# maciejkula/sbr-rs

Hardware: AMD Instinct MI355X
Metric: train interactions/sec (higher is better)
Workload: dtype f32

## Files before the change

### sbr_rs_amd/csrc/sbr_kernels.hip

```cpp

#include "sbr_kernels.h"

#include <atomic>
#include <cstdlib>
#include <cstring>

#include "../../include/sbr_hip.h"
#include "sbr_device.h"
#include "sbr_numerics.h"

namespace sbr {

typedef float f32x4 __attribute__((ext_vector_type(4)));
typedef unsigned v4u32 __attribute__((ext_vector_type(4)));

#define EWMA_CHUNK_SEQS 256
#ifndef SBR_FWD_RT
#define SBR_FWD_RT 4
#endif
#ifndef SBR_FWD_WPE
#define SBR_FWD_WPE 3
#endif
#define SBR_MAX_T 1024
#ifndef SBR_FWD_RT4_MIN_TILES
// ... 1378 lines not shown
        const __amdgpu_buffer_rsrc_t rsC = row_rsrc(w.C, D * 4, rb + b0, nr_live);
#pragma unroll
        for (int k = 0; k < CITER; ++k)
            dst[k] = __builtin_bit_cast(float4, __builtin_amdgcn_raw_buffer_load_b128(rsC, tid * 16, k * NT * 16, SBR_AUX_BWD_LD));
    };
    auto request_gates = [&](int t) {
        const int tid = thread_id();
        int rb, nr;
        step_rows(t, &rb, &nr);
        const __amdgpu_buffer_rsrc_t rsG = row_rsrc(w.G, 4 * D * 4, rb + b0, nr);
        const int vg = (tid / Q) * (4 * D * 4) + (tid % Q) * 16;
#pragma unroll
        for (int k = 0; k < CITER; ++k) {
            const int so = k * (NT / Q) * (4 * D * 4);
#pragma unroll
            for (int g = 0; g < 4; ++g)
                pg[k][g] = __builtin_bit_cast(float4, __builtin_amdgcn_raw_buffer_load_b128(rsG, vg + g * D * 4, so, SBR_AUX_BWD_LD));
        }
    };

    f32x4 ring0[PF], ring1[PF];
    const __amdgpu_buffer_rsrc_t wrs = __builtin_amdgcn_make_buffer_rsrc((void*)m.WTp, (short)0, 2 * D * NGD * 4, SBR_BUFFER_RSRC_FLAGS);
    const uint32_t lane_byte = (uint32_t)(tid0 & 63) * 16u;
    auto load_ring = [&](int slot, int S) {
        ring0[slot] = __builtin_bit_cast(f32x4, __builtin_amdgcn_raw_buffer_load_b128(wrs, lane_byte, (wv * NSZ + S) * 1024, 0));
        ring1[slot] = __builtin_bit_cast(f32x4, __builtin_amdgcn_raw_buffer_load_b128(wrs, lane_byte, ((UT + wv) * NSZ + S) * 1024, 0));
    };
    const int ts = nsteps - 1;
    request_ids(ts);
    request_gates(ts);
    request_cstate(pc, ts);
    request_cstate(pcp, ts > 0 ? ts - 1 : 0);
    request_gathers(ts);
    if (ts > 0) request_ids(ts - 1);
#pragma unroll
    for (int j = 0; j < PF; ++j) load_ring(j, j);

#ifdef SBR_PROF_BWD
    long long bprof[8] = {0, 0, 0, 0, 0, 0, 0, 0};
#define BPROF(k_) { const long long now_ = clock64(); bprof[k_] += now_ - bprof_t; bprof_t = now_; }
    long long bprof_t = clock64();
#else
#define BPROF(k_)
#endif
    auto step = [&](int t) {
        int row_begin, nrows, nrows_above = 0;
        step_rows(t, &row_begin, &nrows);
        if (t + 1 < nsteps) { int rb_; step_rows(t + 1, &rb_, &nrows_above); }
        BPROF(0)
        __syncthreads();
        BPROF(1)
        {
            const int tid = thread_id();
            const __amdgpu_buffer_rsrc_t rsZ = row_rsrc(w.dZ, NGD * 4, row_begin + b0, nrows);
            const int vz = (tid / Q) * (NGD * 4) + (tid % Q) * 16;
#pragma unroll
            for (int k = 0; k < CITER; ++k) {
                const int idx = tid + k * NT;
                const int i = idx / Q;
                const int u = (idx % Q) * 4;
                const bool carried = i < nrows_above;
                const float2 r01 = *reinterpret_cast<const float2*>(&Zs[i * LDZ + u]);
                const float2 r23 = *reinterpret_cast<const float2*>(&Zs[i * LDZ + u + 2]);
                const float recv[4] = {carried ? r01.x : 0.0f, carried ? r01.y : 0.0f, carried ? r23.x : 0.0f, carried ? r23.y : 0.0f};
                const float g_ = pcoef[k];
                const float dhl[4] = {g_ * pen[k].x - g_ * pep[k].x, g_ * pen[k].y - g_ * pep[k].y,
                                      g_ * pen[k].z - g_ * pep[k].z, g_ * pen[k].w - g_ * pep[k].w};
                const float gi[4] = {pg[k][0].x, pg[k][0].y, pg[k][0].z, pg[k][0].w};
                const float gf[4] = {pg[k][1].x, pg[k][1].y, pg[k][1].z, pg[k][1].w};
                const float gg[4] = {pg[k][2].x, pg[k][2].y, pg[k][2].z, pg[k][2].w};
                const float go[4] = {pg[k][3].x, pg[k][3].y, pg[k][3].z, pg[k][3].w};
                const float cc[4] = {pc[k].x, pc[k].y, pc[k].z, pc[k].w};
                const float cp[4] = {pcp[k].x, pcp[k].y, pcp[k].z, pcp[k].w};
                float dz[4][4];
#pragma unroll
                for (int j = 0; j < 4; ++j) {
                    const float dh = dhl[j] + recv[j];
                    float dco;
                    sbr_lstm_cell_bwd(dh, carried ? dc[k][j] : 0.0f, gi[j], gf[j], gg[j], go[j], cc[j], t > 0 ? cp[j] : 0.0f, NG == 3,
                                      &dz[0][j], &dz[1][j], &dz[2][j], &dz[3][j], &dco);
                    dc[k][j] = dco;
                }
#pragma unroll
                for (int g = 0; g < NG; ++g) {
                    const int src = NG == 4 ? g : g + 1;
                    __builtin_amdgcn_raw_buffer_store_b128(__builtin_bit_cast(v4u32, make_float4(dz[src][0], dz[src][1], dz[src][2], dz[src][3])), rsZ,
                                                           vz + g * D * 4, k * (NT / Q) * (NGD * 4), SBR_AUX_BWD_Z);
                    float2* dst = reinterpret_cast<float2*>(&Zs[i * LDZ + g * D + u]);
                    dst[0] = make_float2(dz[src][0], dz[src][1]);
                    dst[1] = make_float2(dz[src][2], dz[src][3]);
                }
            }
        }
        BPROF(2)
        __syncthreads();
        BPROF(3)
        const int tid = thread_id();
        const int lane = tid & 63;
        const int c16 = lane & 15;
        const int kq = lane >> 4;
        f32x4 acc[2][RT];
#pragma unroll
        for (int cc = 0; cc < 2; ++cc)
#pragma unroll
            for (int rt = 0; rt < RT; ++rt) acc[cc][rt] = (f32x4){0.f, 0.f, 0.f, 0.f};
        float av[RT][4];
        auto read_a = [&](int S) {
#pragma unroll
            for (int rt = 0; rt < RT; ++rt) {
                const float* arow = &Zs[(rt * 16 + c16) * LDZ + 16 * (S < NSZ ? S : NSZ - 1) + kq];
                av[rt][0] = arow[0]; av[rt][1] = arow[4]; av[rt][2] = arow[8]; av[rt][3] = arow[12];
            }
        };
        read_a(0);
        auto mma_block = [&](int S, int slot) {
            float ac[RT][4];
#pragma unroll
            for (int rt = 0; rt < RT; ++rt)
#pragma unroll
                for (int sub = 0; sub < 4; ++sub) ac[rt][sub] = av[rt][sub];
            read_a(S + 1);
#pragma unroll
            for (int sub = 0; sub < 4; ++sub)
#pragma unroll
                for (int rt = 0; rt < RT; ++rt) {
                    acc[0][rt] = __builtin_amdgcn_mfma_f32_16x16x4f32(ac[rt][sub], ring0[slot][sub], acc[0][rt], 0, 0, 0);
                    acc[1][rt] = __builtin_amdgcn_mfma_f32_16x16x4f32(ac[rt][sub], ring1[slot][sub], acc[1][rt], 0, 0, 0);
                }
        };
#pragma unroll
        for (int j = 0; j < PF; ++j) {
            mma_block(j, j);
            __builtin_amdgcn_sched_barrier(0);
            load_ring(j, j + PF);
            __builtin_amdgcn_sched_barrier(0);
        }
        if (t > 0) {
            request_gathers(t - 1);
            request_ids(t > 1 ? t - 2 : 0);
        }
        __builtin_amdgcn_sched_barrier(0);
#pragma unroll 1
        for (int S0 = PF; S0 < NSZ - PF; S0 += PF) {
#pragma unroll
            for (int j = 0; j < PF; ++j) {
                mma_block(S0 + j, j);
                __builtin_amdgcn_sched_barrier(0);
                load_ring(j, S0 + j + PF);
                __builtin_amdgcn_sched_barrier(0);
            }
        }
#pragma unroll
        for (int j = 0; j < PF; ++j) {
            mma_block(NSZ - PF + j, j);
            __builtin_amdgcn_sched_barrier(0);
        }
        {
            const int tn = t > 0 ? t - 1 : 0;
#pragma unroll
            for (int k = 0; k < CITER; ++k) pc[k] = pcp[k];
            request_gates(tn);
            request_cstate(pcp, tn > 0 ? tn - 1 : 0);
        }
        BPROF(4)
        __syncthreads();
        BPROF(5)
        {
            const __amdgpu_buffer_rsrc_t rsX = row_rsrc(blk.dX, D * 4, row_begin + b0, nrows);
            const int vx = (kq * 4 * D + wv * 16 + c16) * 4;
#pragma unroll
            for (int rt = 0; rt < RT; ++rt)
#pragma unroll
                for (int reg = 0; reg < 4; ++reg) {
                    const int i = rt * 16 + kq * 4 + reg;
                    const float dx = acc[0][rt][reg];
                    __builtin_amdgcn_raw_buffer_store_b32(__builtin_bit_cast(unsigned, dx), rsX, vx, (rt * 16 + reg) * D * 4, SBR_AUX_BWD_ST);
                    Zs[i * LDZ + wv * 16 + c16] = acc[1][rt][reg];
                }
        }
#pragma unroll
        for (int j = 0; j < PF; ++j) load_ring(j, j);
    };
    step(ts);
#pragma unroll 1
    for (int t = ts - 1; t >= 0; --t) step(t);
#ifdef SBR_PROF_BWD
    if ((tile == 20 || tile == 350) && (tid0 & 63) == 0 && (wv == 0 || wv == 5))
        printf("BWDPROF tile %d wave %d steps %d per-step cycles: epilogue+ringreq %lld barA %lld cell %lld barB %lld gemm+requests %lld barC %lld\n", tile, wv,
               nsteps, bprof[0] / nsteps, bprof[1] / nsteps, bprof[2] / nsteps, bprof[3] / nsteps, bprof[4] / nsteps, bprof[5] / nsteps);
#endif
}

template <int D, int NG>
__global__ __launch_bounds__(256) void lstm_dw_kernel(ModelView m, MbView mb, BlockView blk, WorkView w) {
    constexpr int K2 = 2 * D;
    constexpr int NGD = NG * D;
    constexpr int TJ = (NGD + 127) / 128;
    constexpr int SLAB = 32;
    __shared__ float Xs[SLAB * 128];
    __shared__ float Zs[SLAB * 128];
    __shared__ int s_prev[SBR_DW_CHUNK_ROWS];
    const int tid = threadIdx.x;
    const int lane = tid & 63;
    const int wave = __builtin_amdgcn_readfirstlane(tid >> 6);
    const int wk = wave >> 1, wj = wave & 1;
    constexpr int NTILE = ((K2 + 127) / 128) * TJ;
    const int wid = blockIdx.x;
    const int tile = (wid >> 3) % NTILE;
    const int c = (wid >> 3) / NTILE * 8 + (wid & 7);
    if (c * SBR_DW_CHUNK_ROWS >= mb.R) return;
    const int tk = tile / TJ, tj = tile % TJ;
    const int r0 = c * SBR_DW_CHUNK_ROWS;
    int r1 = r0 + SBR_DW_CHUNK_ROWS;
    if (r1 > mb.R) r1 = mb.R;
    const int nr = r1 - r0;
    for (int i = tid; i < nr; i += 256) {
        s_prev[i] = mb.prev_row[r0 + i];
    }
    __syncthreads();
    const int l31 = lane & 31;
    const int hh = lane >> 5;
    f32x16 acc[2][2];
#pragma unroll
    for (int a = 0; a < 2; ++a)
#pragma unroll
        for (int b = 0; b < 2; ++b)
#pragma unroll
            for (int q = 0; q < 16; ++q) acc[a][b][q] = 0.0f;
    const int c4 = (tid & 31) * 4;
    const int srow = tid >> 5;
    const int kcol = tk * 128 + c4;
    const int jcol = tj * 128 + c4;
    float4 xr[4], zr[4];
    auto fetch = [&](int slab) {
#pragma unroll
        for (int i = 0; i < 4; ++i) {
            const int lr = slab * SLAB + srow + 8 * i;
            float4 xv = make_float4(0.f, 0.f, 0.f, 0.f), zv = make_float4(0.f, 0.f, 0.f, 0.f);
            if (lr < nr) {
                if (kcol < D) xv = ld4(w.X + (size_t)(r0 + lr) * D + kcol);
                else if (kcol < K2) {
                    const int pr = s_prev[lr];
                    if (pr >= 0) xv = ld4(blk.H + (size_t)pr * D + (kcol - D));
                }
                if (jcol < NGD) zv = ld4(w.dZ + (size_t)(r0 + lr) * NGD + jcol);
            }
            xr[i] = xv;
            zr[i] = zv;
        }
    };
    const int nslabs = (nr + SLAB - 1) / SLAB;
    float bias_acc = 0.0f;
    const bool do_bias = tk == 0 && tid < 128 && tj * 128 + tid < NGD;
    fetch(0);
    for (int slab = 0; slab < nslabs; ++slab) {
#pragma unroll
        for (int i = 0; i < 4; ++i) {
            st4(&Xs[(srow + 8 * i) * 128 + c4], xr[i]);
            st4(&Zs[(srow + 8 * i) * 128 + c4], zr[i]);
        }
        __syncthreads();
        if (slab + 1 < nslabs) fetch(slab + 1);
        const float* xa = &Xs[hh * 128 + wk * 64 + l31];
        const float* zb = &Zs[hh * 128 + wj * 64 + l31];
#pragma unroll 4
        for (int s = 0; s < SLAB / 2; ++s) {
            const float a0 = xa[s * 256], a1 = xa[s * 256 + 32];
            const float b0 = zb[s * 256], b1 = zb[s * 256 + 32];
            acc[0][0] = __builtin_amdgcn_mfma_f32_32x32x2f32(a0, b0, acc[0][0], 0, 0, 0);
            acc[0][1] = __builtin_amdgcn_mfma_f32_32x32x2f32(a0, b1, acc[0][1], 0, 0, 0);
            acc[1][0] = __builtin_amdgcn_mfma_f32_32x32x2f32(a1, b0, acc[1][0], 0, 0, 0);
            acc[1][1] = __builtin_amdgcn_mfma_f32_32x32x2f32(a1, b1, acc[1][1], 0, 0, 0);
        }
        if (do_bias) {
            const int rows_here = nr - slab * SLAB < SLAB ? nr - slab * SLAB : SLAB;
            for (int r = 0; r < rows_here; ++r) bias_acc = bias_acc + Zs[r * 128 + tid];
        }
        __syncthreads();
    }
    if (do_bias) w.partials[((size_t)c * (K2 + 1) + K2) * NGD + tj * 128 + tid] = bias_acc;
    float* part = w.partials + (size_t)c * (K2 + 1) * NGD;
#pragma unroll
    for (int a = 0; a < 2; ++a)
#pragma unroll
        for (int b = 0; b < 2; ++b) {
            const int j = tj * 128 + wj * 64 + b * 32 + l31;
#pragma unroll
            for (int q = 0; q < 16; ++q) {
                const int k = tk * 128 + wk * 64 + a * 32 + (q & 3) + 8 * (q >> 2) + 4 * hh;
                if (k < K2 && j < NGD) part[(size_t)k * NGD + j] = acc[a][b][q];
            }
        }
}

template <int D, int NG>
__global__ __launch_bounds__(256, SBR_DW_WPE) void lstm_dw_full_kernel(ModelView m, MbView mb, BlockView blk, WorkView w) {
    constexpr int K2 = 2 * D;
    constexpr int NGD = NG * D;
    constexpr int TJ = NGD / 128;
    constexpr int SLAB = SBR_DW_SLAB;
    constexpr int NI = SLAB / 8;
    constexpr int NTILE = (K2 / 128) * TJ;
    static_assert(K2 % 128 == 0 && NGD % 128 == 0, "full tiles only");
    __shared__ float Xs[SLAB * 128];
    __shared__ float Zs[SLAB * 128];
    __shared__ int s_prev[SBR_DW_CHUNK_ROWS];
    const int tid = threadIdx.x;
    const int lane = tid & 63;
    const int wave = __builtin_amdgcn_readfirstlane(tid >> 6);
    const int wk = wave >> 1, wj = wave & 1;
    const int wid = blockIdx.x;
    const int tile = (wid >> 3) % NTILE;
    const int c = (wid >> 3) / NTILE * 8 + (wid & 7);
    if (c * SBR_DW_CHUNK_ROWS >= mb.R) return;
    const int tk = tile / TJ, tj = tile % TJ;
    const int r0 = c * SBR_DW_CHUNK_ROWS;
    const int last = mb.R - 1;
    for (int i = tid; i < SBR_DW_CHUNK_ROWS; i += 256) s_prev[i] = mb.prev_row[r0 + i <= last ? r0 + i : last];
    __syncthreads();
    const int l31 = lane & 31;
    const int hh = lane >> 5;
    f32x16 acc[2][2];
#pragma unroll
    for (int a = 0; a < 2; ++a)
#pragma unroll
        for (int b = 0; b < 2; ++b)
#pragma unroll
            for (int q = 0; q < 16; ++q) acc[a][b][q] = 0.0f;
    const int c4 = (tid & 31) * 4;
    const int srow = tid >> 5;
    const int kcol = tk * 128 + c4;
    const int jcol = tj * 128 + c4;
    const bool xpart = kcol < D;
    float4 xr[NI], zr[NI];
    const bool small_h = !w.wide_addresses && (size_t)mb.R * D * 4 < ((size_t)1 << 31);
    const int xrows = mb.R - r0 < SBR_DW_CHUNK_ROWS ? mb.R - r0 : SBR_DW_CHUNK_ROWS;
    const __amdgpu_buffer_rsrc_t rsZ = __builtin_amdgcn_make_buffer_rsrc((void*)(w.dZ + (size_t)r0 * NGD), (short)0, xrows * NGD * 4, SBR_BUFFER_RSRC_FLAGS);
    const __amdgpu_buffer_rsrc_t rsXc = __builtin_amdgcn_make_buffer_rsrc((void*)(w.X + (size_t)r0 * D), (short)0, xrows * D * 4, SBR_BUFFER_RSRC_FLAGS);
    const __amdgpu_buffer_rsrc_t rsH = __builtin_amdgcn_make_buffer_rsrc((void*)blk.H, (short)0, small_h ? (int)((size_t)mb.R * D * 4) : 0, SBR_BUFFER_RSRC_FLAGS);
    auto fetch = [&](int slab) {
        if (D >= 128 && small_h) {
#pragma unroll
            for (int i = 0; i < NI; ++i) {
                const int lr = slab * SLAB + srow + 8 * i;
                if (tk * 128 < D) {
                    xr[i] = __builtin_bit_cast(float4, __builtin_amdgcn_raw_buffer_load_b128(rsXc, (srow * D + kcol) * 4, (slab * SLAB + 8 * i) * D * 4, SBR_AUX_DW_LD));
                } else {
                    const int pr = s_prev[lr];
                    xr[i] = __builtin_bit_cast(float4, __builtin_amdgcn_raw_buffer_load_b128(rsH, pr >= 0 ? (int)((uint32_t)pr * (uint32_t)(D * 4) + (uint32_t)((kcol - D) * 4)) : -16, 0, 0));
                }
                zr[i] = __builtin_bit_cast(float4, __builtin_amdgcn_raw_buffer_load_b128(rsZ, (srow * NGD + jcol) * 4, (slab * SLAB + 8 * i) * NGD * 4, SBR_AUX_DW_LD));
            }
            return;
        }
        const float* X = launder(w.X);
        const float* H = launder(blk.H);
        const float* dZ = launder(w.dZ);
        const float* zero = launder(w.zeros);
#pragma unroll
        for (int i = 0; i < NI; ++i) {
            const int lr = slab * SLAB + srow + 8 * i;
            const int row = r0 + lr <= last ? r0 + lr : last;
            const int pr = s_prev[lr];
            const float* src = xpart ? X + ((size_t)row * D + kcol) : (pr >= 0 ? H + ((size_t)pr * D + (kcol - D)) : zero + (kcol - D));
            xr[i] = ld4(src);
            zr[i] = ld4(dZ + ((size_t)(r0 + lr) * NGD + jcol));
        }
    };
    int nr = mb.R - r0;
    nr = nr < SBR_DW_CHUNK_ROWS ? nr : SBR_DW_CHUNK_ROWS;
    const int nslabs = (nr + SLAB - 1) / SLAB;
    float bias_acc = 0.0f;
    const bool do_bias = tk == 0 && tid < 128;
    fetch(0);
    for (int slab = 0; slab < nslabs; ++slab) {
#pragma unroll
        for (int i = 0; i < NI; ++i) {
            st4(&Xs[(srow + 8 * i) * 128 + c4], xr[i]);
            st4(&Zs[(srow + 8 * i) * 128 + c4], zr[i]);
        }
        __syncthreads();
        fetch(slab + 1 < nslabs ? slab + 1 : slab);
        const float* xa = &Xs[hh * 128 + wk * 64 + l31];
        const float* zb = &Zs[hh * 128 + wj * 64 + l31];
        float a0 = xa[0], a1 = xa[32], b0 = zb[0], b1 = zb[32];
#pragma unroll
        for (int s = 0; s < SLAB / 2; ++s) {
            const int sn = s + 1 < SLAB / 2 ? s + 1 : s;
            const float na0 = xa[sn * 256], na1 = xa[sn * 256 + 32];
            const float nb0 = zb[sn * 256], nb1 = zb[sn * 256 + 32];
            acc[0][0] = __builtin_amdgcn_mfma_f32_32x32x2f32(a0, b0, acc[0][0], 0, 0, 0);
            acc[0][1] = __builtin_amdgcn_mfma_f32_32x32x2f32(a0, b1, acc[0][1], 0, 0, 0);
            acc[1][0] = __builtin_amdgcn_mfma_f32_32x32x2f32(a1, b0, acc[1][0], 0, 0, 0);
            acc[1][1] = __builtin_amdgcn_mfma_f32_32x32x2f32(a1, b1, acc[1][1], 0, 0, 0);
            a0 = na0; a1 = na1; b0 = nb0; b1 = nb1;
        }
        if (do_bias) {
            const int rows_here = nr - slab * SLAB < SLAB ? nr - slab * SLAB : SLAB;
            for (int r = 0; r < rows_here; ++r) bias_acc = bias_acc + Zs[r * 128 + tid];
        }
        __syncthreads();
    }
    if (do_bias) w.partials[((size_t)c * (K2 + 1) + K2) * NGD + tj * 128 + tid] = bias_acc;
    float* part = w.partials + (size_t)c * (K2 + 1) * NGD;
#pragma unroll
    for (int a = 0; a < 2; ++a)
#pragma unroll
        for (int b = 0; b < 2; ++b) {
            const int j = tj * 128 + wj * 64 + b * 32 + l31;
#pragma unroll
            for (int q = 0; q < 16; ++q) {
                const int k = tk * 128 + wk * 64 + a * 32 + (q & 3) + 8 * (q >> 2) + 4 * hh;
                part[(size_t)k * NGD + j] = acc[a][b][q];
            }
        }
}

__global__ void dense_reduce_local_kernel(const float* partials, int nchunks, size_t n, float* dense) {
    const size_t i = (size_t)blockIdx.x * blockDim.x + threadIdx.x;
    if (i >= n) return;
    float acc = partials[i];
    int c = 1;
    for (; c + 8 <= nchunks; c += 8) {
        float v[8];
#pragma unroll
        for (int j = 0; j < 8; ++j) v[j] = partials[(size_t)(c + j) * n + i];
#pragma unroll
        for (int j = 0; j < 8; ++j) acc = acc + v[j];
    }
    for (; c < nchunks; ++c) acc = acc + partials[(size_t)c * n + i];
    dense[i] = acc;
}

__device__ __forceinline__ size_t wp_index(int k, int jcol, int D, int NG) {
    const int K2 = 2 * D;
    const int g = jcol / D, u = jcol % D;
    const int ut = u >> 4, j16 = u & 15;
    const int S = k >> 4, sub = (k & 15) >> 2, kq = k & 3;
    const int lane = kq * 16 + j16;
    return ((((size_t)(ut * NG + g) * (K2 / 16) + S) * 64 + lane) * 4 + sub);
}
__device__ __forceinline__ size_t wtp_index(int k, int jcol, int D, int NG) {
    const int NGD = NG * D;
    const int ct = k >> 4, c16 = k & 15;
    const int S = jcol >> 4, sub = (jcol & 15) >> 2, kq = jcol & 3;
    const int lane = kq * 16 + c16;
    return ((((size_t)ct * (NGD / 16) + S) * 64 + lane) * 4 + sub);
}

__device__ __forceinline__ void dense_apply_element(const ModelView& m, size_t i, float g);
__global__ void dense_apply_kernel(ModelView m, const uint8_t* all_blocks, uint64_t block_bytes, uint64_t dense_off,
                                   int ndev, size_t n, const float* partials, int nchunks, float* dense_out) {
    const size_t i = (size_t)blockIdx.x * blockDim.x + threadIdx.x;
    if (i >= n) return;
    float g;
    if (partials) {
        g = partials[i];
        int c = 1;
        for (; c + 8 <= nchunks; c += 8) {
            float v[8];
#pragma unroll
            for (int j = 0; j < 8; ++j) v[j] = partials[(size_t)(c + j) * n + i];
#pragma unroll
            for (int j = 0; j < 8; ++j) g = g + v[j];
        }
        for (; c < nchunks; ++c) g = g + partials[(size_t)c * n + i];
        dense_out[i] = g;
    } else {
        g = reinterpret_cast<const float*>(all_blocks + dense_off)[i];
        for (int q = 1; q < ndev; ++q) g = g + reinterpret_cast<const float*>(all_blocks + (size_t)q * block_bytes + dense_off)[i];
    }
    dense_apply_element(m, i, g);
}
__device__ __forceinline__ void dense_apply_element(const ModelView& m, size_t i, float g) {
    if (m.ng) {
        const int NGD = m.ng * m.d;
        const size_t nw = (size_t)2 * m.d * NGD;
        if (i < nw) {
            const bool adam = m.optimizer == SBR_OPT_ADAM;
            float wv = m.W[i], G = m.Wacc[i], M = adam ? m.Wm[i] : 0.0f;
            opt_update(m, &wv, &G, &M, g);
            m.W[i] = wv;
            m.Wacc[i] = G;
            if (adam) m.Wm[i] = M;
            const int k = (int)(i / NGD), jcol = (int)(i % NGD);
            m.Wp[wp_index(k, jcol, m.d, m.ng)] = wv;
            m.WTp[wtp_index(k, jcol, m.d, m.ng)] = wv;
        } else {
            const size_t j = i - nw;
            const bool adam = m.optimizer == SBR_OPT_ADAM;
            float wv = m.bW[j], G = m.bWacc[j], M = adam ? m.bWm[j] : 0.0f;
            opt_update(m, &wv, &G, &M, g);
            m.bW[j] = wv;
            m.bWacc[j] = G;
            if (adam) m.bWm[j] = M;
        }
    } else {
        const bool adam = m.optimizer == SBR_OPT_ADAM;
        float wv = m.alpha[i], G = m.alpha_acc[i], M = adam ? m.alpha_m[i] : 0.0f;
        opt_update(m, &wv, &G, &M, g);
        m.alpha[i] = wv;
        m.alpha_acc[i] = G;
        if (adam) m.alpha_m[i] = M;
    }
}

__global__ void repack_lstm_kernel(ModelView m) {
    const int NGD = m.ng * m.d;
    const size_t nw = (size_t)2 * m.d * NGD;
    const size_t i = (size_t)blockIdx.x * blockDim.x + threadIdx.x;
    if (i >= nw) return;
    const int k = (int)(i / NGD), jcol = (int)(i % NGD);
    const float wv = m.W[i];
    m.Wp[wp_index(k, jcol, m.d, m.ng)] = wv;
    m.WTp[wtp_index(k, jcol, m.d, m.ng)] = wv;
}


struct UpdAccess {
    static __device__ __forceinline__ float4 ld(const float* p) { return ld4_upd(p); }
    static __device__ __forceinline__ void st(float* p, float4 v) { st4_upd(p, v); }
};
struct NoPrefetch {};
struct EmitApply {
    ModelView m;
    template <int D>
    __device__ __forceinline__ RowUpdate<D> pre(uint32_t r, int lg) const {
        RowUpdate<D> q;
        q.template load<UpdAccess>(m, r, lg);
        return q;
    }
    template <int D>
    __device__ __forceinline__ void row(uint32_t r, uint64_t, int lg, const RowSum& s, RowUpdate<D> q) const {
        q.apply(m, s);
        q.template store<UpdAccess>(m, r, lg);
        q.update_bias(m, r, lg, s);
    }
};
struct EmitChunk {
    void* send;
    uint64_t S;
    template <int D>
    __device__ __forceinline__ NoPrefetch pre(uint32_t, int) const { return NoPrefetch{}; }
    template <int D>
    __device__ __forceinline__ void row(uint32_t r, uint64_t, int lg, const RowSum& s, NoPrefetch) const {
        const uint32_t S32 = (uint32_t)S, owner = r / S32;
        float* c = reinterpret_cast<float*>(send) + (uint64_t)owner * S * ((uint64_t)D + 2);
        const uint64_t lr = r - owner * S32;
        st4(c + lr * D + 4 * lg, s.g);
        if (lg == 0) {
            if (s.has_b()) c[S * D + lr] = s.gb;
            reinterpret_cast<uint32_t*>(c + S * D + S)[lr] = 1u | (s.has_b() ? 2u : 0u);
        }
    }
};
struct EmitList {
    float* G;
    float* gbl;
    uint32_t* fl;
    template <int D>
    __device__ __forceinline__ NoPrefetch pre(uint32_t, int) const { return NoPrefetch{}; }
    template <int D>
    __device__ __forceinline__ void row(uint32_t, uint64_t p, int lg, const RowSum& s, NoPrefetch) const {
        st4(G + p * D + 4 * lg, s.g);
        if (lg == 0) {
            gbl[p] = s.gb;
            fl[p] = 1u | (s.has_b() ? 2u : 0u);
        }
    }
};

template <int D>
__device__ __forceinline__ RowSum seg_accumulate(const BlockView& blk, const uint64_t* keys, uint64_t begin, uint64_t end, int lg) {
    RowSum s;
    for (uint64_t e = begin; e < end; e += 4) {
        float4 v[4];
        float sc[4];
        bool bias[4];
#pragma unroll
        for (int i = 0; i < 4; ++i) {
            v[i] = make_float4(0.f, 0.f, 0.f, 0.f);
            sc[i] = 0.0f;
            bias[i] = false;
            if (e + i < end) {
                const EntrySource src = entry_source((uint32_t)keys[e + i]);
                v[i] = ld4(src.rows(blk.dX, blk.H) + (size_t)src.r * D + 4 * lg);
                sc[i] = src.scale_at(blk.coef);
                bias[i] = src.carries_bias();
            }
        }
#pragma unroll
        for (int i = 0; i < 4; ++i)
            if (e + i < end) s.add_entry(v[i], sc[i], bias[i]);
    }
    return s;
}

template <int D, int NB>
__device__ __forceinline__ RowSum seg_accumulate_long(const BlockView& blk, const uint64_t* keys, uint64_t begin, uint64_t end, int lg) {
    RowSum s;
    const uint32_t* klo = reinterpret_cast<const uint32_t*>(keys);
    uint32_t src_n[NB];
#pragma unroll
    for (int i = 0; i < NB; ++i) src_n[i] = begin + i < end ? klo[2 * (begin + i)] : 0u;
#pragma unroll 1
    for (uint64_t e = begin; e < end; e += NB) {
        float4 v[NB];
        float sc[NB];
        EntrySource src[NB];
#pragma unroll
        for (int i = 0; i < NB; ++i) {
            src[i] = entry_source(src_n[i]);
            v[i] = make_float4(0.f, 0.f, 0.f, 0.f);
            sc[i] = 0.0f;
            if (e + i < end) {
                v[i] = ld4(src[i].rows(blk.dX, blk.H) + (size_t)src[i].r * D + 4 * lg);
                sc[i] = blk.coef[src[i].r];
            }
        }
#pragma unroll
        for (int i = 0; i < NB; ++i) src_n[i] = e + NB + i < end ? klo[2 * (e + NB + i)] : 0u;
#pragma unroll
        for (int i = 0; i < NB; ++i)
            if (e + i < end) s.add_entry(v[i], src[i].scale(sc[i]), src[i].carries_bias());
    }
    return s;
}

__device__ __forceinline__ uint64_t seg_end(const uint64_t* keys, uint64_t lo, uint64_t hi, uint32_t row) {
    while (lo < hi) {
        const uint64_t mid = lo + (hi - lo) / 2;
        if ((uint32_t)(keys[mid] >> 32) == row) lo = mid + 1; else hi = mid;
    }
    return lo;
}

template <int D, class Emit, bool INLINE_LONG>
__device__ __forceinline__ void seg_short_rows(const BlockView& blk, const uint64_t* keys, uint64_t n, const SegScratch& sc, const Emit& emit,
                                               uint32_t wave, uint32_t nwaves) {
    const LaneGroup<D> lanes(wave, nwaves);
    constexpr int L = LaneGroup<D>::L;
    const int lg = lanes.lg, gbase = lanes.grp * L;
    const uint32_t nheads = *sc.nheads;
    const uint32_t stride = (uint32_t)lanes.stride;
    uint32_t h = (uint32_t)lanes.first();
    auto head_at = [&](uint32_t hh) { return sc.head_pos[hh < nheads ? hh : nheads]; };
    auto window_key = [&](uint32_t p0, uint32_t p1) {
        const uint32_t c = p1 - p0 < (uint32_t)L ? p1 - p0 : (uint32_t)L;
        return keys[(uint32_t)lg < c ? (uint64_t)p0 + lg : ((uint64_t)p0 < n ? (uint64_t)p0 : 0)];
    };
    uint32_t p_cur = head_at(h), p_end = head_at(h + 1);
    uint32_t p_next = head_at(h + stride), p_next_end = head_at(h + stride + 1);
    uint64_t kmine = window_key(p_cur, p_end);
    for (uint32_t h0 = (uint32_t)lanes.wave_first; h0 < nheads; h0 += stride, h += stride) {
        const bool active = h < nheads;
        const uint32_t p_nn = head_at(h + 2 * stride), p_nn_end = head_at(h + 2 * stride + 1);
        const uint64_t p = p_cur;
        const uint32_t len = active ? p_end - p_cur : 0u;
        const uint32_t cnt = len < (uint32_t)L ? len : (uint32_t)L;
        const uint32_t lo = (uint32_t)kmine;
        const uint32_t row = (uint32_t)__shfl((int)(uint32_t)(kmine >> 32), gbase, 64);
        kmine = window_key(p_next, p_next_end);
        p_cur = p_next;
        p_end = p_next_end;
        p_next = p_nn;
        p_next_end = p_nn_end;
        if (INLINE_LONG && len > SBR_SEG_CHUNK) {
            const auto pre = emit.template pre<D>(row, lg);
            RowSum s = seg_accumulate_long<D, 8>(blk, keys, p, p + SBR_SEG_CHUNK, lg);
            for (uint64_t q = p + SBR_SEG_CHUNK; q < p + len; q += SBR_SEG_CHUNK)
                s.add_partial(seg_accumulate_long<D, 8>(blk, keys, q, q + SBR_SEG_CHUNK < p + len ? q + SBR_SEG_CHUNK : p + len, lg));
            emit.template row<D>(row, p, lg, s, pre);
            continue;
        }
        if (!INLINE_LONG && len > SBR_SEG_ROUTE) {
            if (lg == 0 && !sc.prelisted) {
                const uint32_t slot = atomicAdd(&sc.counters[0], 1u);
                if (slot < sc.cap) {
                    sc.long_start[slot] = (uint32_t)p;
                    sc.long_end[slot] = (uint32_t)p + len;
                }
            }
            continue;
        }
        if (!active) continue;
        const auto pre = emit.template pre<D>(row, lg);
        RowSum s;
        if (len <= (uint32_t)L) {
            for (int e = 0; e < (int)cnt; e += 4) {
                float4 v[4];
                float scl[4];
                bool bias[4];
#pragma unroll
                for (int i = 0; i < 4; ++i) {
                    v[i] = make_float4(0.f, 0.f, 0.f, 0.f);
                    scl[i] = 0.0f;
                    bias[i] = false;
                    if (e + i < (int)cnt) {
                        const EntrySource src = entry_source((uint32_t)__shfl((int)lo, gbase + e + i, 64));
                        v[i] = ld4(src.rows(blk.dX, blk.H) + (size_t)src.r * D + 4 * lg);
                        scl[i] = src.scale_at(blk.coef);
                        bias[i] = src.carries_bias();
                    }
                }
#pragma unroll
                for (int i = 0; i < 4; ++i)
                    if (e + i < (int)cnt) s.add_entry(v[i], scl[i], bias[i]);
            }
        } else {
            s = seg_accumulate<D>(blk, keys, p, p + len, lg);
        }
        emit.template row<D>(row, p, lg, s, pre);
    }
}
template <int D, class Emit, bool INLINE_LONG = false>
__global__ __launch_bounds__(256) void seg_short_kernel(BlockView blk, const uint64_t* keys, uint64_t n, SegScratch sc, Emit emit) {
    seg_short_rows<D, Emit, INLINE_LONG>(blk, keys, n, sc, emit, (uint32_t)((blockIdx.x * (uint64_t)blockDim.x + threadIdx.x) >> 6),
                                         (uint32_t)(((uint64_t)gridDim.x * blockDim.x) >> 6));
// ... 881 lines not shown
```

Before: 108.6 million.

## Switch LSTM dW kernel to 16x16x4 MFMA with padded LDS rows

Replaces the 2x2 grid of 32x32x2 f32 MFMAs in the full-tile LSTM weight-gradient kernel with a 4x4 grid of 16x16x4 MFMAs that consume four k-rows per step. LDS rows are padded to a stride of 144 floats so fragment reads avoid bank conflicts, and the output store is rewritten to match the new accumulator layout. It also adds optional compile-time scheduling barriers and a hoisted bias reduction. The goal is higher MFMA throughput and fewer LDS conflicts, at the cost of more accumulator registers and more shared memory.

After: 109.1 million (median of 6 runs). About the same (+0.4%).

```diff
diff --git a/sbr_rs_amd/csrc/sbr_kernels.hip b/sbr_rs_amd/csrc/sbr_kernels.hip
--- a/sbr_rs_amd/csrc/sbr_kernels.hip
+++ b/sbr_rs_amd/csrc/sbr_kernels.hip
@@ -1704,8 +1704,10 @@
     constexpr int NI = SLAB / 8;
     constexpr int NTILE = (K2 / 128) * TJ;
     static_assert(K2 % 128 == 0 && NGD % 128 == 0, "full tiles only");
-    __shared__ float Xs[SLAB * 128];
-    __shared__ float Zs[SLAB * 128];
+    constexpr int LD = 144;
+    static_assert(SLAB % 4 == 0 && LD % 32 == 16, "whole k-blocks per slab; conflict-free fragment reads");
+    __shared__ float Xs[SLAB * LD];
+    __shared__ float Zs[SLAB * LD];
     __shared__ int s_prev[SBR_DW_CHUNK_ROWS];
     const int tid = threadIdx.x;
     const int lane = tid & 63;
@@ -1720,15 +1722,15 @@
     const int last = mb.R - 1;
     for (int i = tid; i < SBR_DW_CHUNK_ROWS; i += 256) s_prev[i] = mb.prev_row[r0 + i <= last ? r0 + i : last];
     __syncthreads();
-    const int l31 = lane & 31;
-    const int hh = lane >> 5;
-    f32x16 acc[2][2];
-#pragma unroll
-    for (int a = 0; a < 2; ++a)
-#pragma unroll
-        for (int b = 0; b < 2; ++b)
-#pragma unroll
-            for (int q = 0; q < 16; ++q) acc[a][b][q] = 0.0f;
+    const int j16 = lane & 15;
+    const int kq = lane >> 4;
+    f32x4 acc[4][4];
+#pragma unroll
+    for (int a = 0; a < 4; ++a)
+#pragma unroll
+        for (int b = 0; b < 4; ++b)
+#pragma unroll
+            for (int q = 0; q < 4; ++q) acc[a][b][q] = 0.0f;
     const int c4 = (tid & 31) * 4;
     const int srow = tid >> 5;
     const int kcol = tk * 128 + c4;
@@ -1778,44 +1780,73 @@
     for (int slab = 0; slab < nslabs; ++slab) {
 #pragma unroll
         for (int i = 0; i < NI; ++i) {
-            st4(&Xs[(srow + 8 * i) * 128 + c4], xr[i]);
-            st4(&Zs[(srow + 8 * i) * 128 + c4], zr[i]);
+            st4(&Xs[(srow + 8 * i) * LD + c4], xr[i]);
+            st4(&Zs[(srow + 8 * i) * LD + c4], zr[i]);
         }
         __syncthreads();
         fetch(slab + 1 < nslabs ? slab + 1 : slab);
-        const float* xa = &Xs[hh * 128 + wk * 64 + l31];
-        const float* zb = &Zs[hh * 128 + wj * 64 + l31];
-        float a0 = xa[0], a1 = xa[32], b0 = zb[0], b1 = zb[32];
-#pragma unroll
-        for (int s = 0; s < SLAB / 2; ++s) {
-            const int sn = s + 1 < SLAB / 2 ? s + 1 : s;
-            const float na0 = xa[sn * 256], na1 = xa[sn * 256 + 32];
-            const float nb0 = zb[sn * 256], nb1 = zb[sn * 256 + 32];
-            acc[0][0] = __builtin_amdgcn_mfma_f32_32x32x2f32(a0, b0, acc[0][0], 0, 0, 0);
-            acc[0][1] = __builtin_amdgcn_mfma_f32_32x32x2f32(a0, b1, acc[0][1], 0, 0, 0);
-            acc[1][0] = __builtin_amdgcn_mfma_f32_32x32x2f32(a1, b0, acc[1][0], 0, 0, 0);
-            acc[1][1] = __builtin_amdgcn_mfma_f32_32x32x2f32(a1, b1, acc[1][1], 0, 0, 0);
-            a0 = na0; a1 = na1; b0 = nb0; b1 = nb1;
+        const float* xa = &Xs[kq * LD + wk * 64 + j16];
+        const float* zb = &Zs[kq * LD + wj * 64 + j16];
+        float av[4], bv[4];
+#pragma unroll
+        for (int f = 0; f < 4; ++f) {
+            av[f] = xa[16 * f];
+            bv[f] = zb[16 * f];
+        }
+#pragma unroll
+        for (int s = 0; s < SLAB / 4; ++s) {
+            const int sn = s + 1 < SLAB / 4 ? s + 1 : s;
+            float na[4], nb[4];
+#pragma unroll
+            for (int f = 0; f < 4; ++f) {
+                na[f] = xa[sn * 4 * LD + 16 * f];
+                nb[f] = zb[sn * 4 * LD + 16 * f];
+            }
+#if SBR_DW_ORDERED == 1
+            __builtin_amdgcn_sched_barrier(0);
+#endif
+#pragma unroll
+            for (int a = 0; a < 4; ++a)
+#pragma unroll
+                for (int b = 0; b < 4; ++b) acc[a][b] = __builtin_amdgcn_mfma_f32_16x16x4f32(av[a], bv[b], acc[a][b], 0, 0, 0);
+#if SBR_DW_ORDERED == 1
+            __builtin_amdgcn_sched_barrier(0);
+#elif SBR_DW_ORDERED == 2
+#pragma unroll
+            for (int g = 0; g < 4; ++g) {
+                __builtin_amdgcn_sched_group_barrier(0x008, 2, 0);
+                __builtin_amdgcn_sched_group_barrier(0x100, 1, 0);
+            }
+            __builtin_amdgcn_sched_group_barrier(0x008, 8, 0);
+#endif
+#pragma unroll
+            for (int f = 0; f < 4; ++f) {
+                av[f] = na[f];
+                bv[f] = nb[f];
+            }
         }
         if (do_bias) {
+#if SBR_DW_BIAS_HOIST
+            float zv[SLAB];
+#pragma unroll
+            for (int r = 0; r < SLAB; ++r) zv[r] = Zs[r * LD + tid];
+#pragma unroll
+            for (int r = 0; r < SLAB; ++r) bias_acc = bias_acc + zv[r];
+#else
             const int rows_here = nr - slab * SLAB < SLAB ? nr - slab * SLAB : SLAB;
-            for (int r = 0; r < rows_here; ++r) bias_acc = bias_acc + Zs[r * 128 + tid];
+            for (int r = 0; r < rows_here; ++r) bias_acc = bias_acc + Zs[r * LD + tid];
+#endif
         }
         __syncthreads();
     }
     if (do_bias) w.partials[((size_t)c * (K2 + 1) + K2) * NGD + tj * 128 + tid] = bias_acc;
-    float* part = w.partials + (size_t)c * (K2 + 1) * NGD;
-#pragma unroll
-    for (int a = 0; a < 2; ++a)
-#pragma unroll
-        for (int b = 0; b < 2; ++b) {
-            const int j = tj * 128 + wj * 64 + b * 32 + l31;
-#pragma unroll
-            for (int q = 0; q < 16; ++q) {
-                const int k = tk * 128 + wk * 64 + a * 32 + (q & 3) + 8 * (q >> 2) + 4 * hh;
-                part[(size_t)k * NGD + j] = acc[a][b][q];
-            }
-        }
+    float* part = w.partials + ((size_t)c * (K2 + 1) + tk * 128 + wk * 64 + 4 * kq) * NGD + tj * 128 + wj * 64 + j16;
+#pragma unroll
+    for (int a = 0; a < 4; ++a)
+#pragma unroll
+        for (int q = 0; q < 4; ++q)
+#pragma unroll
+            for (int b = 0; b < 4; ++b) part[(size_t)(16 * a + q) * NGD + 16 * b] = acc[a][b][q];
 }
 
 __global__ void dense_reduce_local_kernel(const float* partials, int nchunks, size_t n, float* dense) {
```
